# fnordware/j2k

Hardware: AMD Instinct MI355X
Metric: Mpixels/s encode, 8Kx8K 16-bit RGB, 5 DWT levels; DWT HBM GB/s vs roofline (higher is better)
Workload: dtype f32

## Files before the change

j2k_amd/csrc/encoder.cpp:

```cpp
#include <hip/hip_runtime.h>

#include <dlfcn.h>

#include <algorithm>
#include <atomic>
#include <chrono>
#include <condition_variable>
#include <functional>
#include <future>
#include <limits>
#include <cstdio>
#include <cstdlib>
#include <cstring>
#include <memory>
#include <mutex>
#include <thread>
#include <string>
#include <vector>

#include "common.h"
#include "geometry.h"
#include "kernels.h"
#include "tier2.h"
#include "jp2.h"
// ... 469 lines not shown
    std::unique_lock<std::mutex> dense(dev.dense);
    const unsigned dense_seq = ++dev.seq;
    unsigned *const dwt_word = dev.dwt_done_word;
    unsigned *const dwt_busy = (dwt_word && tn.mq_yield && tn.overlap && dev.inflight.load() > 1) ? dwt_word + 32 : nullptr;
    const size_t nb1 = g.cblks.size();
    const size_t nb = nb1 * F;
    const T1Tables tt(nb);
    e->sym.ensure(e->sym_bytes * F + 1024);
    e->out.ensure(e->out_bytes * F + 64);
    e->meta.ensure(tt.meta_bytes());
    e->passes.ensure(tt.passes_bytes());
    HIP_CHECK(hipMemsetAsync(tt.err(e->meta.as<uint32_t>()), 0, sizeof(uint32_t), s));

    const bool overlap_mq = tn.overlap != 0;
    if (overlap_mq && dev.last_dense_done && dev.last_dense_done != e->k1_done) HIP_CHECK(hipStreamWaitEvent(s, dev.last_dense_done, 0));
    HIP_CHECK(hipEventRecord(e->ev[EV_UPLOAD], s));

    const size_t plane_bytes = e->frame_elems * sizeof(int32_t);
    FrontendArgs fa0 = make_frontend_args(cod, dplanes, x0, y0, x1, y1);
    const bool fused = fuse_frontend(cod, fa0, tn);
    if (!fused || NL >= 3) e->P.ensure(plane_bytes * F);
    if (NL >= 1) e->Z.ensure(plane_bytes * F);
    if (NL >= 2) e->Q.ensure(plane_bytes * F);
    const bool level_events = tn.level_events != 0;
    double dwt_bytes = 0;
    struct BusyGuard {
        unsigned *word = nullptr; hipStream_t s;
        ~BusyGuard() { if (word) (void)hipMemsetAsync(word, 0, sizeof(unsigned), s); }
    } busy_guard;
    busy_guard.s = s;
    for (size_t f = 0; f < F; ++f) {
    if (f > 0) for (uint32_t c = 0; c < cod.ncomp; ++c) dplanes[c] = planes[f * cod.ncomp + c];
    FrontendArgs fa = f == 0 ? fa0 : make_frontend_args(cod, dplanes, x0, y0, x1, y1);
    if (!fused) {
        fa.dst_x0 = x0; fa.dst_y0 = y0;
        run_frontend(e, cod, fa, reinterpret_cast<int32_t *>(e->P.as<uint8_t>() + f * plane_bytes), e->comp_off, S, s);
    }
    if (f == 0) e->last_fa = fa;
    if (f == 0) HIP_CHECK(hipEventRecord(e->ev[EV_FRONT], s));

    if (f == 0 && dwt_busy && NL > 0) { launch_set_word(dwt_busy, 1u, s); busy_guard.word = dwt_busy; }
    const bool own_bracket = f == 0 && F == 1 && NL > 0 && tn.level1_dispatch_events;
    if (f == 0 && !own_bracket) HIP_CHECK(hipEventRecord(e->lev[0], s));
    for (int l = 0; l < NL; ++l) {
        const int l1 = l + 1;
        const bool last_own = own_bracket && !level_events && l > 0 && l == NL - 1;
        const bool bracketed = (l == 0 && own_bracket) || last_own;
        launch_dwt_levels(e, cod, fa, fused, f, l, l1, s, bracketed ? e->lev[l] : nullptr, bracketed ? e->lev[l1] : nullptr);
        HIP_CHECK(hipGetLastError());
        for (const DwtJob &j : e->h_jobs[(size_t)l]) dwt_bytes += 8.0 * j.rw * j.rh;
        if (!bracketed && ((F == 1 && level_events) || (l == 0 && F == 1) || (l1 == NL && f == F - 1))) HIP_CHECK(hipEventRecord(e->lev[l1], s));
        if (l == 0 && f == 0 && busy_guard.word && tn.mq_yield == 1 && NL > 1) { launch_set_word(dwt_busy, 0u, s); busy_guard.word = nullptr; }
    }
    }
    e->last_levels = NL;
    e->last_fused = fused;
    const bool word_by_modeller = dwt_word && !busy_guard.word;
    if (dwt_word && !word_by_modeller) launch_set_word(dwt_word, dense_seq, s, busy_guard.word, 0u);
    busy_guard.word = nullptr;
    HIP_CHECK(hipEventRecord(e->ev[EV_DWT], s));

    if (F > 1 && (e->seq_frames != F || !e->seq_valid)) {
        e->h_blks_seq.resize(nb);
        for (size_t f = 0; f < F; ++f)
            for (size_t i = 0; i < nb1; ++i) {
                CblkDev d = e->h_blks[i];
                d.coef_off += (unsigned long long)f * e->frame_elems;
                d.sym_off += (unsigned long long)f * e->sym_bytes;
                d.out_off += (unsigned long long)f * e->out_bytes;
                e->h_blks_seq[f * nb1 + i] = d;
            }
        e->blks_seq.ensure(nb * sizeof(CblkDev));
        HIP_CHECK(hipMemcpyAsync(e->blks_seq.p, e->h_blks_seq.data(), nb * sizeof(CblkDev), hipMemcpyHostToDevice, s));
        e->seq_frames = F; e->seq_valid = true;
    }
    const CblkDev *dblk = F > 1 ? e->blks_seq.as<CblkDev>() : e->blks.as<CblkDev>();
    uint32_t *meta = e->meta.as<uint32_t>();
    T1Args ta{};
    ta.coef = NL >= 1 ? e->Z.p : e->P.p; ta.stride = (long long)S;
    ta.blks = dblk; ta.nblks = (int)nb; ta.reversible = cod.reversible;
    t1_arena_args(e, tt, ta);
    ta.mq_prio = tn.mq_prio ? 3 : 0;
    ta.sparse = tn.t1_sparse;
    ta.style = cod.cblk_style;
#ifdef J2K_MQ_TIMES
    {
        static unsigned long long *dbg = nullptr;
        if (!dbg) { HIP_CHECK(hipMalloc(reinterpret_cast<void **>(&dbg), kT1Counters * 8)); }
        else {
            unsigned long long h[12];
            HIP_CHECK(hipMemcpy(h, dbg, sizeof(h), hipMemcpyDeviceToHost));
            const double ch = (double)std::max(1ull, h[4]), wv = (double)std::max(1ull, h[5]);
            std::fprintf(stderr, "coder waves (previous frame): %.0f workgroups, %.0f chunks each; per chunk of 16 decisions, counter ticks: producer work %.1f + barrier %.1f | "
                                 "consumer work %.1f + barrier %.1f\n", wv, ch / wv, h[0] / ch, h[1] / ch, h[2] / ch, h[3] / ch);
        }
        HIP_CHECK(hipMemset(dbg, 0, kT1Counters * 8));
        ta.dbg = dbg;
    }
#endif
#ifdef J2K_T1_COUNTERS
    t1_counters(ta);
#endif
    ta.yield_word = (dwt_word && tn.mq_yield && tn.overlap) ? dwt_word + 32 : nullptr;
    const bool rate_control = cod.rate_control();
    ta.want_dist = rate_control ? 1 : 0;
    ta.want_rates = rate_control ? 1 : 0;
    {
        const int big_groups = std::max(2, std::min(7, tn.groups));
        const int groups = nb >= 8192 ? big_groups : 1;
        int first = 0;
        for (int gi = 0; gi < groups; ++gi) {
            const size_t eighth = (nb / 8) / 64 * 64;
            int last = gi == groups - 1 ? (int)nb : (int)((eighth + (nb - eighth) * (size_t)gi / (size_t)(groups - 1)) / 64 * 64);
            T1Args tg = ta;
            tg.first = first; tg.nblks = last;
            if (gi == 0 && word_by_modeller) { tg.done_word = dwt_word; tg.done_value = dense_seq; }
            launch_t1_model(tg, s);
            {
                HIP_CHECK(hipEventRecord(e->gev[gi], s));
                HIP_CHECK(hipStreamWaitEvent(coder_stream(e, gi), e->gev[gi], 0));
                if (tn.mq_wait_us > 0 && dwt_word && overlap_mq && gi == groups - 1 && groups > 1 && dev.inflight.load() > 1)
                    launch_wait_word(dwt_word, dense_seq + 1, (unsigned)tn.mq_wait_us, e->mqs[gi]);
                launch_t1_mq(tg, e->mqs[gi]);
                HIP_CHECK(hipEventRecord(e->mq_done[gi], e->mqs[gi]));
            }
            first = last;
        }
        HIP_CHECK(hipEventRecord(e->k1_done, s));
        for (int gi = 0; gi < groups; ++gi) HIP_CHECK(hipStreamWaitEvent(s, e->mq_done[gi], 0));
    }
    HIP_CHECK(hipEventRecord(e->ev[EV_T1], s));

    e->h_meta.ensure(tt.meta_bytes());
    HIP_CHECK(hipMemcpyAsync(e->h_meta.p, meta, tt.meta_words() * sizeof(uint32_t), hipMemcpyDeviceToHost, s));
    if (rate_control && nb) {
        T1Args tf = ta;
        tf.first = 0; tf.nblks = (int)nb;
        launch_t1_rate_fixup(tf, s);
        e->h_passes.ensure(tt.h_passes_bytes());
        const int dev_min = tn.rate_dev == 0 ? 8192 : tn.rate_dev;
        pd.rc_device = dev_min > 0 && cod.psnr.empty() && F == 1 && nb >= (size_t)dev_min && (!cod.max_comp_size || dev.inflight.load() <= 1);
        pd.rc_tables_pending = false;
        if (!(pd.rc_device && tn.overlap))
            HIP_CHECK(hipMemcpyAsync(e->h_passes.p, ta.pass_nmsedec, tt.h_passes_bytes(), hipMemcpyDeviceToHost, s));
        if (pd.rc_device) {
            const RateArgs ra = rate_args(e, tt);
            if (!e->rc_weight_valid) {
                const std::vector<double> w = rate_block_weights(g);
                std::memcpy(e->h_rc_bounds.p, w.data(), nb * sizeof(double));
                unsigned char *hc = e->h_rc_bounds.as<unsigned char>() + nb * sizeof(double);
                for (size_t i = 0; i < nb; ++i) hc[i] = (unsigned char)std::min<uint32_t>(g.cblks[i].comp, 3u);
                HIP_CHECK(hipMemcpyAsync(e->rc_weight.p, e->h_rc_bounds.p, nb * sizeof(double) + nb, hipMemcpyHostToDevice, s));
                e->rc_weight_valid = true;
            }
            launch_rate_prepare(ra, s);
            if (tn.overlap) {
                hipStream_t side = coder_stream(e, 0);
                HIP_CHECK(hipEventRecord(e->rc_fixed, s));
                HIP_CHECK(hipStreamWaitEvent(side, e->rc_fixed, 0));
                HIP_CHECK(hipMemcpyAsync(e->h_passes.p, ta.pass_nmsedec, tt.h_passes_bytes(), hipMemcpyDeviceToHost, side));
                HIP_CHECK(hipEventRecord(e->rc_tables, side));
                pd.rc_tables_pending = true;
            }
            HIP_CHECK(hipMemcpyAsync(e->h_rc_bounds.p, ra.bounds, 3 * nb * sizeof(double), hipMemcpyDeviceToHost, s));
        }
    } else {
// ... 237 lines not shown
    for (int k = 0; k < j2k_hip_encoder::kMaxStages; ++k) {
        if (!e->stage_done[k]) HIP_CHECK(hipEventCreateWithFlags(&e->stage_done[k], hipEventDisableTiming));
        if (!e->stage_dl[k]) HIP_CHECK(hipEventCreateWithFlags(&e->stage_dl[k], hipEventDisableTiming));
    }
    if (!e->band_valid || e->band_row_end != rows) {
        e->band = build_band_schedule(g, rows, split_last);
        e->band_row_end = rows;
        e->h_blks_band.resize(nb);
        size_t sym_off = 0, out_off = 0;
        for (size_t n = 0; n < nb; ++n) {
            CblkDev d = e->h_blks[e->band.perm[n]];
            d.sym_off = sym_off; d.out_off = out_off;
            sym_off += d.sym_cap; out_off += d.out_cap;
            e->h_blks_band[n] = d;
        }
        e->blks_band.ensure(nb * sizeof(CblkDev));
        e->pack_dst.ensure(nb * sizeof(unsigned long long));
        HIP_CHECK(hipMemcpyAsync(e->blks_band.p, e->h_blks_band.data(), nb * sizeof(CblkDev), hipMemcpyHostToDevice, s));
        const BandSchedule &Sn = e->band;
        const int nst = (int)Sn.stages.size(), nbands = (int)rows.size();
        e->h_gate_groups.clear(); e->h_group_of.assign(nb, 0);
        e->stage_group_first.assign((size_t)nst, 0); e->stage_group_count.assign((size_t)nst, 0);
        for (int k = 0; k < nst; ++k) {
            const BandStage &st = Sn.stages[(size_t)k];
            e->stage_group_first[(size_t)k] = (uint32_t)e->h_gate_groups.size();
            const unsigned prio = (st.band == nbands - 1 && nbands > 1) ? 3u : (2 * st.band >= nbands - 1 ? 2u : 1u);
            for (uint32_t f = 0; f < st.blk_count; f += 64) {
                const uint32_t cnt = std::min<uint32_t>(64, st.blk_count - f);
                for (uint32_t i = 0; i < cnt; ++i) e->h_group_of[st.blk_first + f + i] = (uint32_t)e->h_gate_groups.size();
                e->h_gate_groups.push_back(T1Args::GateGroup{st.blk_first + f, cnt, (unsigned)k, prio});
            }
            e->stage_group_count[(size_t)k] = (uint32_t)e->h_gate_groups.size() - e->stage_group_first[(size_t)k];
        }
        e->gate_groups.ensure(std::max<size_t>(1, e->h_gate_groups.size()) * sizeof(T1Args::GateGroup));
        e->gate_group_of.ensure(nb * sizeof(uint32_t));
        if (!e->h_gate_groups.empty())
            HIP_CHECK(hipMemcpyAsync(e->gate_groups.p, e->h_gate_groups.data(), e->h_gate_groups.size() * sizeof(T1Args::GateGroup), hipMemcpyHostToDevice, s));
        HIP_CHECK(hipMemcpyAsync(e->gate_group_of.p, e->h_group_of.data(), nb * sizeof(uint32_t), hipMemcpyHostToDevice, s));
        HIP_CHECK(hipStreamSynchronize(s));
        e->band_valid = true;
    }
    const BandSchedule &S = e->band;
    const int NS = (int)S.stages.size();
    if (NS > j2k_hip_encoder::kMaxStages) throw Error(J2K_HIP_ERR_PARAM, "internal: more stages than events");
    const size_t NG = e->h_gate_groups.size();

    const size_t pad = reinterpret_cast<uintptr_t>(lo) & 15;
    e->in.ensure(span + pad + 16);
    uint8_t *const dbase = e->in.as<uint8_t>() + pad;
    const size_t plane_bytes = e->plane_elems * sizeof(int32_t) * cod.ncomp;
    if (NL >= 3) e->P.ensure(plane_bytes);
    e->Z.ensure(plane_bytes);
    if (NL >= 2) e->Q.ensure(plane_bytes);
    e->sym.ensure(e->sym_bytes + 1024);
    e->out.ensure(e->out_bytes + 64);
    e->cs.ensure(e->out_bytes + 64);
    const T1Tables tt(nb);
    e->meta.ensure(tt.meta_bytes());
    e->passes.ensure(tt.passes_bytes());
    e->h_meta.ensure(tt.meta_bytes());
    uint32_t *meta = e->meta.as<uint32_t>();
    e->gate_state.ensure((NG + (size_t)NS + 8) * sizeof(uint32_t));
    unsigned *const gate_ready = e->gate_state.as<unsigned>(), *const gate_done = gate_ready + NG, *const gate_abort = gate_done + NS;
    HIP_CHECK(hipEventRecord(e->ev[EV_START], s));
    HIP_CHECK(hipMemsetAsync(tt.err(meta), 0, sizeof(uint32_t), s));
    HIP_CHECK(hipMemsetAsync(gate_ready, 0, (NG + (size_t)NS + 8) * sizeof(uint32_t), s));
    HIP_CHECK(hipEventRecord(e->gates_zeroed, s));

    j2k_hip_plane dplanes[4];
    for (uint32_t c = 0; c < cod.ncomp; ++c) {
        dplanes[c] = planes[c];
        dplanes[c].base = dbase + (static_cast<const uint8_t *>(planes[c].base) - lo);
    }
    const FrontendArgs fa = make_frontend_args(cod, dplanes, 0, 0, (int)cod.width, (int)cod.height);
    e->last_fa = fa; e->last_fused = true; e->last_levels = NL;
    for (int l = 0; l < NL; ++l) e->level_ms[l] = 0;

    T1Args ta{};
    ta.coef = e->Z.p; ta.stride = (long long)e->stride;
    ta.blks = e->blks_band.as<CblkDev>(); ta.nblks = (int)nb; ta.reversible = cod.reversible;
    t1_arena_args(e, tt, ta);
    ta.mq_prio = tn.mq_prio ? 3 : 0;
    ta.sparse = tn.t1_sparse;
    ta.want_rates = 0;
    ta.gate_groups = e->gate_groups.as<T1Args::GateGroup>(); ta.gate_group_of = e->gate_group_of.as<unsigned>();
    ta.gate_ready = gate_ready; ta.gate_done = gate_done; ta.gate_abort = gate_abort;
    ta.gate_budget = 1u << 21;

    double dwt_bytes = 0;
    for (int l = 0; l < NL; ++l)
        for (const DwtJob &j : e->h_jobs[(size_t)l]) dwt_bytes += 8.0 * j.rw * j.rh;

    pd.banded = true;
    HIP_CHECK(hipStreamWaitEvent(s_coder, e->gates_zeroed, 0));
    for (size_t g0 = 0; g0 < NG; g0 += 1024) launch_t1_mq_gated(ta, (int)g0, (int)std::min<size_t>(1024, NG - g0), s_coder);
    double up_ms = 0;
    for (int k = 0; k < NS; ++k) {
        const BandStage &st = S.stages[(size_t)k];
        if (k < B) {
            Range r("j2k_hip upload band");
            const uint8_t *b0 = k ? lo + (size_t)rows[(size_t)k - 1] * (size_t)rowbytes : lo;
            const uint8_t *b1 = k == B - 1 ? hi : std::min(hi, lo + (size_t)rows[(size_t)k] * (size_t)rowbytes);
            const double t0 = now_ms();
            if (b1 > b0) HIP_CHECK(hipMemcpyAsync(dbase + (b0 - lo), b0, (size_t)(b1 - b0), hipMemcpyHostToDevice, e->up_stream));
            up_ms += now_ms() - t0;
            HIP_CHECK(hipEventRecord(e->band_up[k], e->up_stream));
        }
        Range r("j2k_hip band enqueue");
        if (k < B) HIP_CHECK(hipStreamWaitEvent(s, e->band_up[k], 0));
        for (const BandLaunch &bl : st.dwt) {
            DwtLevelArgs da = dwt_level_args(e, cod, fa, true, 0, (int)bl.level, (int)bl.tile_row);
            da.pair0 = bl.pair0; da.pair1 = bl.pair1;
            launch_dwt_level(da, s);
        }
        HIP_CHECK(hipGetLastError());
        if (k < B) {
            HIP_CHECK(hipEventRecord(e->gev[k], s));
            uint32_t first = st.blk_first, count = st.blk_count;
            if (k == B - 1) for (int q = B; q < NS; ++q) count += S.stages[(size_t)q].blk_count;
            if (count) {
                T1Args tg = ta;
                tg.first = (int)first; tg.nblks = (int)(first + count);
                tg.model_prio = (k == B - 1 && B > 1) ? 3 : 0;
                HIP_CHECK(hipStreamWaitEvent(s_model, e->gev[k], 0));
                launch_t1_model(tg, s_model);
            }
        }
    }
    HIP_CHECK(hipEventSynchronize(e->band_up[B - 1]));
    pd.t_uploaded = now_ms();
    for (int k = 0; k < NS; ++k) {
        const BandStage &st = S.stages[(size_t)k];
        if (st.blk_count) {
            launch_wait_count(gate_done + k, e->stage_group_count[(size_t)k], 10000000u, gate_abort, ta.err, e->dl_stream);
            unsigned long long *pd_dst = e->pack_dst.as<unsigned long long>() + st.blk_first;
            launch_pack_offsets(ta.len + st.blk_first, (int)st.blk_count, e->h_blks_band[st.blk_first].out_off, pd_dst, e->dl_stream);
            GatherArgs ga{};
            ga.dst = e->cs.as<uint8_t>(); ga.out = e->out.as<uint8_t>(); ga.blks = ta.blks + st.blk_first;
            ga.cblk_dst = pd_dst; ga.len = ta.len + st.blk_first; ga.nblks = (int)st.blk_count;
            launch_gather(ga, e->dl_stream);
            HIP_CHECK(hipMemcpy2DAsync(tt.numbps(e->h_meta.as<uint32_t>()) + st.blk_first, tt.column_bytes(), tt.numbps(meta) + st.blk_first, tt.column_bytes(),
                                       st.blk_count * sizeof(uint32_t), T1Tables::kColumns, hipMemcpyDeviceToHost, e->dl_stream));
        }
        HIP_CHECK(hipEventRecord(e->stage_done[k], e->dl_stream));
    }


    for (int k = 0; k < NS; ++k) HIP_CHECK(hipStreamWaitEvent(s, e->stage_done[k], 0));
    HIP_CHECK(hipMemcpyAsync(tt.err(e->h_meta.as<uint32_t>()), tt.err(meta), sizeof(uint32_t), hipMemcpyDeviceToHost, s));
    HIP_CHECK(hipEventRecord(e->ev[EV_T1], s));

    pd.active = true;
    pd.F = 1; pd.nb1 = nb; pd.framed = true; pd.rate_control = false; pd.dwt_bytes = dwt_bytes;
    pd.meta = meta; pd.dblk = ta.blks; pd.nl = NL;
    pd.banded = true; pd.stages = NS; pd.bands = B; pd.ms_upload_host = up_ms;
    return true;
}

struct PieceWriter {
    j2k_hip_write_fn write; void *user; std::vector<uint8_t> &bounce; size_t fill = 0;
    static constexpr size_t kSmall = 256u << 10, kBounce = 4u << 20;
    void out(const uint8_t *p, size_t n) { if (n && write(user, p, n) != n) throw Error(J2K_HIP_ERR_SINK, "Error writing file"); }
    void flush() { if (fill) { out(bounce.data(), fill); fill = 0; } }
    void put(const uint8_t *p, size_t n)
    {
        if (n >= kSmall) { flush(); out(p, n); return; }
// ... 673 lines not shown
```

j2k_amd/csrc/kernels.h:

```cpp
#pragma once

#include <hip/hip_runtime.h>

#include <cstdint>

#include "rgba_plan.h"

namespace j2k_hip {

struct Tuning {
    int overlap = 1;
    int no_fuse = 0;
    int level_events = 0;
    int level1_dispatch_events = 1;
    int mq_prio = 1;
    int mq_yield = 2;
    int groups = 2;
    int alloc_threads = 8;
    int rate_dev = 0;
    int rate_dev_scan = 0;
    int mq_wait_us = 1500;
    int dwt_pairs = 2;
    int dwt_ppc = 0;
    int dwt_min_waves = 2048;
    int fused_wpb = 0;
    int fused_ppc = 0;
    int fused_generic = 0;
    int dwt_xcd = 1;
    int t1dec_tail = 1;
    int t1dec_lanes = 1;
    int decseq_group = 0;
    int bands = 0;
    int t1_sparse = 0;
};
Tuning &tuning();
int tune(const char *key, int value);
int get_tune(const char *key, int *value);

struct FrontendArgs {
    const uint8_t *src[4];
    long long colbytes[4], rowbytes[4];
    int sample_bytes[4];
    int src_depth[4];
    int ncomp;
    int width;
    int x0;
    int y0, y1;
    int dst_x0, dst_y0;
    int prec;
    int reversible, mct, promote;
    int interleaved;
    const uint8_t *pixel_base;
    int pixel_bytes;
    int chan_off[4];
    void *dst[4];
    long long dst_stride;
    const float *xyz_lin[3];
    const float *xyz_thr;
    float xyz_m[9];
};
void launch_frontend(const FrontendArgs &a, hipStream_t s);
void launch_frontend_sycc(const FrontendArgs &a, int sub_x, int sub_y, hipStream_t s);
void launch_frontend_xyz(const FrontendArgs &a, hipStream_t s);

constexpr int kCompareWords = 8;
constexpr int kCompareSets = 16;
struct CompareArgs {
    FrontendArgs src;
    int wide;
    const int *planes[4]; long long plane_stride; int plane_dc;
    const uint16_t *dec[4]; long long dec_stride[4]; int dec_sx[4], dec_sy[4];
    int ncomp, width, height;
    int slot[4];
    unsigned long long *acc;
};
void launch_compare(const CompareArgs &a, hipStream_t s);

struct DwtJob {
    long long src_off;
    long long ll_off;
    long long z_off;
    int rw, rh;
    int casx, casy;
    int px0, py0;
};
struct DwtLevelArgs {
    const void *src; long long src_stride;
    void *ll; long long ll_stride;
    void *z; long long z_stride;
    const DwtJob *jobs; int njobs;
    int max_rw, max_rh;
    int reversible;
    int pair0, pair1;
    int shared_chip;
    int fused;
    long long comp_stride;
    struct Fused {
        const uint8_t *base;
        long long rowbytes;
        int pixb;
        int k0, k1, k2, k3;
        int rs;
        int dc;
        int mct;
        int ncomp;
        int promote;
        int src_depth, prec;
    } fe;
};
void launch_dwt_level(const DwtLevelArgs &a, hipStream_t s, hipEvent_t start = nullptr, hipEvent_t stop = nullptr);
int fused_occupancy(bool rev, int ncomp);
void launch_membw(const void *src, void *dst, int w, int h, int rows, int mode, hipStream_t s);

struct CblkDev {
    unsigned long long coef_off;
    unsigned long long sym_off;
    unsigned long long out_off;
    unsigned int sym_cap, out_cap;
    float stepsize;
    unsigned short w, h;
    unsigned char orient, Mb;
    unsigned char pad[2];
};
constexpr int kDevMaxPasses = 96;
constexpr int kT1Counters = 56;
struct T1Args {
    const void *coef; long long stride;
    const CblkDev *blks; int nblks;
    int first;
    int reversible;
    int want_dist;
    int want_rates;
    int mq_prio;
    int model_prio;
    int sparse;
#if defined(J2K_T1_COUNTERS) || defined(J2K_MQ_TIMES)
    unsigned long long *dbg;
#endif
    unsigned *done_word; unsigned done_value;
    struct GateGroup { unsigned first, count, stage, prio; };
    const GateGroup *gate_groups;
    const unsigned *gate_group_of;
    unsigned *gate_ready, *gate_done;
    const unsigned *gate_abort;
    unsigned gate_budget;
    const unsigned *yield_word;
    uint8_t *sym;
    uint8_t *out;
    unsigned int *numbps, *npasses, *nsym, *len, *err;
    unsigned int *pass_nsym;
    int *pass_nmsedec;
    unsigned int *pass_rate;
    unsigned style;
};
void launch_t1_model(const T1Args &a, hipStream_t s);
void launch_t1_mq(const T1Args &a, hipStream_t s);
void launch_t1_mq_styled(const T1Args &a, hipStream_t s);
void launch_t1_mq_gated(const T1Args &a, int group_first, int group_count, hipStream_t s);
void launch_wait_count(const unsigned *word, unsigned target, unsigned timeout_us, const unsigned *abort, unsigned *err, hipStream_t s);
void launch_wait_word(const unsigned *word, unsigned target, unsigned timeout_us, hipStream_t s);
void launch_set_word(unsigned *word, unsigned value, hipStream_t s, unsigned *word2 = nullptr, unsigned value2 = 0);
void launch_t1_rate_fixup(const T1Args &a, hipStream_t s);

struct Taken;
struct RateArgs {
    unsigned nblks;
    const double *weight;
    const unsigned char *comp_of;
    const unsigned *numbps, *npasses;
    const int *pass_nmsedec;
    const unsigned *pass_rate;
    double *disto;
    float *reach;
    double *bounds;
    const unsigned char *done;
    const double *ahead;
    long long *delta;
    unsigned *scan_bytes;
    Taken *scan_taken;
    unsigned long long *scan_sums;
};
void launch_rate_prepare(const RateArgs &a, hipStream_t s);
void launch_rate_ahead(const RateArgs &a, unsigned first, unsigned count, unsigned K, hipStream_t s);
void launch_rate_scan(const RateArgs &a, unsigned first, unsigned count, double thresh, hipStream_t s);

struct DecBlkDev {
    unsigned long long cw_off;
    unsigned long long mask_off;
    unsigned long long coef_off;
    unsigned int cw_len;
    float stepsize;
    unsigned short w, h, npasses;
    unsigned char orient, numbps;
    unsigned int seg_off;
    unsigned short nsegs;
    unsigned char roishift;
};
struct DecGroupDev {
    unsigned long long plane_off;
    unsigned maxpasses, maxstripes;
};
struct T1DecArgs {
    const uint8_t *cw;
    unsigned long long *masks;
    void *coef; long long stride;
    const DecBlkDev *blks; int nblks;
    int reversible;
    const DecGroupDev *groups;
    unsigned *state, *planes;
    const unsigned *cwsegs;
    unsigned style;
#ifdef T1L_STATS
    unsigned long long *stats;
#endif
};
void launch_t1_decode(const T1DecArgs &a, hipStream_t s);
void launch_t1_decode_lanes(const T1DecArgs &a, hipStream_t s);
int t1_decode_lanes_resident_waves();

struct IdwtJob {
    long long off;
    int rw, rh;
    int casx, casy;
};
struct IdwtArgs {
    void *a, *tmp; long long stride;
    const IdwtJob *jobs; int njobs;
    int max_rw, max_rh;
    int reversible;
};
void launch_idwt_level(const IdwtArgs &a, hipStream_t s);

struct IdwtWinJob {
    long long off;
    int rw, rh, casx, casy;
    int wx0, wx1, wy0, wy1;
// ... 52 lines not shown
```

j2k_amd/csrc/stage_hooks.cpp:

```cpp
#include <algorithm>
#include <cstring>
#include <memory>
#include <string>
#include <utility>
#include <vector>

#include "cblk_style.h"
#include "handle.h"
#include "rate_device.h"
#include "tier2.h"

using namespace j2k_hip;

static int stage_t1_blocks(j2k_hip_encoder *e, int reversible, void *d_coef, uint32_t stride, uint32_t nblocks,
                           const uint32_t *bx, const uint32_t *by, const uint32_t *bw, const uint32_t *bh, const uint32_t *orient,
                           const float *stepsize, uint32_t *numbps, uint32_t *npasses, uint32_t *length, uint64_t *offsets,
                           void *data, size_t data_cap, uint32_t *pass_rate, int32_t *pass_dist, uint32_t cblk_style)
{
    if (!e) return J2K_HIP_ERR_PARAM;
    return guarded(e, [&] {
        if (e->pend.active) throw Error(J2K_HIP_ERR_PARAM, "the previous j2k_hip_encode_begin on this handle has not been finished");
        if (cblk_style & kStyleVcausal) throw Error(J2K_HIP_ERR_PARAM, "cblk_style: vertically causal contexts (bit 8) are not written");
        if (cblk_style & ~(uint32_t)(kStylesEncoded | kStyleVcausal)) throw Error(J2K_HIP_ERR_PARAM, "cblk_style: unknown code-block style bits");
        HIP_CHECK(hipSetDevice(e->device));
        hipStream_t s = e->stream;
        const size_t nb = nblocks;
        std::vector<CblkDev> blks(nb);
        size_t sym_off = 0, out_off = 0;
        for (size_t i = 0; i < nb; ++i) {
            if (bw[i] == 0 || bh[i] == 0 || bw[i] > 64 || bh[i] > 64 || orient[i] > 3) throw Error(J2K_HIP_ERR_PARAM, "bad code-block rectangle");
            CblkDev d{};
            d.coef_off = (unsigned long long)by[i] * stride + bx[i];
            const size_t area = (size_t)bw[i] * bh[i];
            const CblkCaps caps = cblk_capacities(area, 30, cblk_style);
            const size_t symcap = caps.sym, outcap = caps.out;
            d.sym_off = sym_off; d.sym_cap = (unsigned)symcap; d.out_off = out_off; d.out_cap = (unsigned)outcap;
            d.stepsize = stepsize ? stepsize[i] : 1.0f;
            d.w = (unsigned short)bw[i]; d.h = (unsigned short)bh[i]; d.orient = (unsigned char)orient[i]; d.Mb = 30;
            sym_off += symcap; out_off += outcap;
            blks[i] = d;
        }
        {
            std::vector<uint32_t> order(nb);
            for (uint32_t i = 0; i < nb; ++i) order[i] = i;
            std::sort(order.begin(), order.end(), [&](uint32_t a, uint32_t b) { return by[a] < by[b]; });
            for (size_t i = 0; i < nb; ++i)
                for (size_t j = i + 1; j < nb && by[order[j]] < by[order[i]] + bh[order[i]]; ++j) {
                    const uint32_t a = order[i], b = order[j];
                    if (bx[a] < bx[b] + bw[b] && bx[b] < bx[a] + bw[a]) throw Error(J2K_HIP_ERR_PARAM, "code-block rectangles overlap");
                }
            for (size_t i = 0; i < nb; ++i)
                if ((uint64_t)bx[i] + bw[i] > stride) throw Error(J2K_HIP_ERR_PARAM, "code-block rectangle wider than the plane's stride");
        }
        invalidate_cached_tables(e);
        const T1Tables tt(nb);
        e->blks.ensure(std::max<size_t>(1, nb) * sizeof(CblkDev));
        if (nb) HIP_CHECK(hipMemcpyAsync(e->blks.p, blks.data(), nb * sizeof(CblkDev), hipMemcpyHostToDevice, s));
        e->sym.ensure(sym_off + 1024); e->out.ensure(out_off + 64);
        e->meta.ensure(tt.meta_bytes());
        e->passes.ensure(tt.passes_bytes());
        T1Args ta{};
        ta.coef = d_coef; ta.stride = stride; ta.blks = e->blks.as<CblkDev>(); ta.nblks = (int)nb; ta.reversible = reversible;
        t1_arena_args(e, tt, ta);
        ta.want_dist = pass_dist != nullptr;
        ta.want_rates = pass_rate || pass_dist;
        ta.sparse = tuning().t1_sparse;
        ta.style = cblk_style;
#ifdef J2K_T1_COUNTERS
        t1_counters(ta);
#endif
        HIP_CHECK(hipMemsetAsync(ta.err, 0, sizeof(uint32_t), s));
        launch_t1_model(ta, s);
        launch_t1_mq(ta, s);
        if (cblk_style) launch_t1_rate_fixup(ta, s);
        std::vector<uint32_t> hm(tt.meta_words());
        HIP_CHECK(hipMemcpyAsync(hm.data(), e->meta.p, hm.size() * sizeof(uint32_t), hipMemcpyDeviceToHost, s));
        HIP_CHECK(hipStreamSynchronize(s));
        if (*tt.err(hm.data())) throw Error(J2K_HIP_ERR_OVERFLOW, "Tier-1 kernel reported error " + std::to_string(*tt.err(hm.data())));
        size_t pos = 0;
        for (size_t i = 0; i < nb; ++i) {
            numbps[i] = tt.numbps(hm.data())[i]; npasses[i] = tt.npasses(hm.data())[i]; length[i] = tt.len(hm.data())[i];
            offsets[i] = pos;
            if (pos + length[i] > data_cap) throw Error(J2K_HIP_ERR_OVERFLOW, "data buffer too small");
            if (length[i]) HIP_CHECK(hipMemcpy(static_cast<uint8_t *>(data) + pos, e->out.as<uint8_t>() + blks[i].out_off, length[i], hipMemcpyDeviceToHost));
            pos += length[i];
        }
        if (pass_rate || pass_dist) {
            std::vector<uint32_t> hp(tt.passes_words());
            HIP_CHECK(hipMemcpy(hp.data(), e->passes.p, hp.size() * sizeof(uint32_t), hipMemcpyDeviceToHost));
            for (size_t i = 0; i < nb; ++i) {
                const uint32_t np = npasses[i];
                uint32_t *rate = tt.pass_rate(hp.data()) + tt.row(i);
                const uint32_t *nmsedec = tt.pass_nmsedec(hp.data()) + tt.row(i);
                if (!cblk_style) {
                    uint32_t last = length[i];
                    for (uint32_t p = np; p > 0;) { --p; if (rate[p] > last) rate[p] = last; else last = rate[p]; }
                    const uint8_t *bytes = static_cast<const uint8_t *>(data) + offsets[i];
                    for (uint32_t p = 0; p < np; ++p)
                        if (rate[p] > 0 && bytes[rate[p] - 1] == 0xff) --rate[p];
                }
                for (uint32_t p = 0; p < (uint32_t)kDevMaxPasses; ++p) {
                    if (pass_rate) pass_rate[tt.row(i) + p] = p < np ? rate[p] : 0;
                    if (pass_dist) pass_dist[tt.row(i) + p] = p < np ? (int32_t)nmsedec[p] : 0;
                }
            }
        }
    });
}

extern "C" {

int j2k_hip_stage_frontend(j2k_hip_encoder *e, const j2k_hip_params *params, const j2k_hip_plane *planes_device, void *d_out)
{
    if (!e) return J2K_HIP_ERR_PARAM;
    return guarded(e, [&] {
        if (e->pend.active) throw Error(J2K_HIP_ERR_PARAM, "the previous j2k_hip_encode_begin on this handle has not been finished");
        HIP_CHECK(hipSetDevice(e->device));
        const Coding cod = normalise(params);
        FrontendArgs fa = make_frontend_args(cod, planes_device, 0, 0, (int)cod.width, (int)cod.height);
        if (cod.subsampled() || cod.rgb_to_sycc || cod.rgb_to_xyz) {
            const PlaneLayout lay = plane_layout(cod, 0, 0, (int)cod.width, (int)cod.height);
            e->P.ensure(lay.frame_elems * sizeof(int32_t));
            run_frontend(e, cod, fa, e->P.as<int32_t>(), lay.comp_off, lay.stride, e->stream);
            HIP_CHECK(hipGetLastError());
            uint8_t *out = static_cast<uint8_t *>(d_out);
            for (uint32_t c = 0; c < cod.ncomp; ++c) {
                const size_t cw = (size_t)lay.cw[c], chh = (size_t)lay.ch[c];
                HIP_CHECK(hipMemcpy2DAsync(out, cw * 4, e->P.as<int32_t>() + lay.comp_off[c], lay.stride * 4, cw * 4, chh, hipMemcpyDeviceToDevice, e->stream));
                out += cw * chh * 4;
            }
            HIP_CHECK(hipStreamSynchronize(e->stream));
            return;
        }
        for (uint32_t c = 0; c < cod.ncomp; ++c) fa.dst[c] = static_cast<int32_t *>(d_out) + (size_t)c * cod.width * cod.height;
        fa.dst_stride = cod.width;
        launch_frontend(fa, e->stream);
        HIP_CHECK(hipStreamSynchronize(e->stream));
    });
}

int j2k_hip_stage_dwt(j2k_hip_encoder *e, int reversible, uint32_t width, uint32_t height, uint32_t nplanes, uint32_t levels,
                      uint32_t x0, uint32_t y0, const void *d_in, void *d_out, uint32_t repeat, double *ms_out)
{
    if (!e) return J2K_HIP_ERR_PARAM;
    return guarded(e, [&] {
        if (e->pend.active) throw Error(J2K_HIP_ERR_PARAM, "the previous j2k_hip_encode_begin on this handle has not been finished");
        HIP_CHECK(hipSetDevice(e->device));
        if (!width || !height || !nplanes || levels > 32) throw Error(J2K_HIP_ERR_PARAM, "bad DWT stage arguments");
        const size_t plane = (size_t)width * height;
// ... 575 lines not shown
```

j2k_amd/csrc/t1.hip:

```cpp
#include "kernels.h"
#include "t1_common.h"
#include "cblk_style.h"

#include <algorithm>
#include <cstdlib>
#include <type_traits>

namespace j2k_hip {
namespace {


constexpr int kFrac = 6;
constexpr int kFlush = 1024;
constexpr int kStageBytes = kFlush + 64 * 10;


__device__ __forceinline__ void set_priority(int p)
{
    if (p >= 3) __builtin_amdgcn_s_setprio(3);
    else if (p == 2) __builtin_amdgcn_s_setprio(2);
    else if (p == 1) __builtin_amdgcn_s_setprio(1);
}

__device__ __forceinline__ unsigned from_left(unsigned v) { return (unsigned)__builtin_amdgcn_update_dpp(0, (int)v, 0x138 , 0xf, 0xf, false); }
__device__ __forceinline__ unsigned from_right(unsigned v) { return (unsigned)__builtin_amdgcn_update_dpp(0, (int)v, 0x130 , 0xf, 0xf, false); }

__device__ __forceinline__ u64 from_left64(u64 v) { return (u64)from_left((unsigned)v) | ((u64)from_left((unsigned)(v >> 32)) << 32); }
__device__ __forceinline__ u64 from_right64(u64 v) { return (u64)from_right((unsigned)v) | ((u64)from_right((unsigned)(v >> 32)) << 32); }

__device__ __forceinline__ unsigned prefix_count_dpp(unsigned cnt, unsigned &total)
{
    int t = (int)cnt;
    t += __builtin_amdgcn_update_dpp(0, t, 0x111, 0xf, 0xf, false);
    t += __builtin_amdgcn_update_dpp(0, t, 0x112, 0xf, 0xf, false);
    t += __builtin_amdgcn_update_dpp(0, t, 0x114, 0xf, 0xf, false);
    t += __builtin_amdgcn_update_dpp(0, t, 0x118, 0xf, 0xf, false);
    t += __builtin_amdgcn_update_dpp(0, t, 0x142, 0xa, 0xf, false);
    t += __builtin_amdgcn_update_dpp(0, t, 0x143, 0xc, 0xf, false);
    total = (unsigned)__builtin_amdgcn_readlane(t, 63);
    return (unsigned)t - cnt;
}

__device__ __forceinline__ unsigned nibble_counts(unsigned v)
{
    const unsigned x = v - ((v >> 1) & 0x55555555u);
    return (x & 0x33333333u) + ((x >> 2) & 0x33333333u);
}

constexpr unsigned kDenseStripe = 103, kSparseHead = 64, kSparseRound = 44;
constexpr unsigned kBurst = 64 * 10;

__device__ __forceinline__ int nmsedec_sig(unsigned m, int bp)
{
    const int i = (int)((m >> bp) & 127u);
    return bp > 0 ? max(0, (3 * i - 144) * 128) : ((i * i + 32) >> 6) * 128;
}
__device__ __forceinline__ int nmsedec_ref(unsigned m, int bp)
{
    const int i = (int)((m >> bp) & 127u);
    if (bp > 0) return i >= 64 ? max(0, (i - 80) * 128) : max(0, (48 - i) * 128);
    return (((i - 64) * (i - 64) + 32) >> 6) * 128;
}

struct PackSel {
    u64 v[256];
    constexpr PackSel() : v()
    {
        for (int e = 0; e < 256; ++e) {
            u64 sel = 0x0c0c0c0c0c0c0c0cull;
            int k = 0;
            for (int r = 0; r < 4; ++r) {
                if ((e >> r) & 1) { sel = (sel & ~(0xffull << (8 * k))) | ((u64)r << (8 * k)); ++k; }
                if ((e >> (4 + r)) & 1) { sel = (sel & ~(0xffull << (8 * k))) | ((u64)(4 + r) << (8 * k)); ++k; }
            }
            v[e] = sel;
        }
    }
};
__constant__ PackSel kPackSel = PackSel();

struct PairTab {
    unsigned v[256];
    constexpr PairTab() : v()
    {
        for (unsigned e = 0; e < 256; ++e) {
// ... 693 lines not shown
#ifdef J2K_MQ_TIMES
        long long tw_ = 0, tb_ = 0;
#endif
        for (unsigned c = 0; c <= nchunks; ++c) {
#ifdef J2K_MQ_TIMES
            const long long t0_ = __builtin_readcyclecounter();
#endif
            if (a.yield_word && (c & 3u) == 0) {
                while (yield_budget && __builtin_amdgcn_readfirstlane((int)__hip_atomic_load(a.yield_word, __ATOMIC_RELAXED, __HIP_MEMORY_SCOPE_AGENT))) {
                    __builtin_amdgcn_s_sleep(64);
                    --yield_budget;
                }
            }
            if (c < nchunks) {
                const unsigned base = c * 16;
                const uint4 chunk = next;
                if (base + 16 < nsym) next = *reinterpret_cast<const uint4 *>(sym + base + 16);
                const unsigned words[4] = {chunk.x, chunk.y, chunk.z, chunk.w};
                const int rem = (int)min(nsym - min(base, nsym), 16u);
                unsigned char *const ctx_b = reinterpret_cast<unsigned char *>(ctxs);
                const unsigned char *const trans_b = reinterpret_cast<const unsigned char *>(trans);
                const unsigned lane4 = (unsigned)lane * 4u;
                auto decide = [&](unsigned c4, unsigned b4, auto jj_) -> unsigned {
                    constexpr unsigned jj = decltype(jj_)::value;
                    unsigned *const cp = reinterpret_cast<unsigned *>(ctx_b + __builtin_amdgcn_perm(c4, lane4, 0x0c0c0400u + (jj << 8)));
                    const unsigned st = *cp;
                    const unsigned ta = (st ^ __builtin_amdgcn_perm(b4, 0u, 0x0c0c040cu + (jj << 8))) & 0x3fcu;
                    const unsigned tr = *reinterpret_cast<const unsigned *>(trans_b + ta);
                    const bool mps = ta < (1u << kMq2LpsBit);
                    const unsigned qe = st & 0xffff0000u;
                    const unsigned A1 = A - qe;
                    const bool use_a1 = (A1 >= qe) == mps;
                    A = use_a1 ? A1 : qe;
                    const bool renorm = (int)A >= 0;
                    *cp = renorm ? tr : st;
                    const unsigned n = (unsigned)__builtin_clz(A);
                    A <<= n;
                    return __builtin_amdgcn_alignbit(n, use_a1 ? qe : 0u, 16);
                };
                if (__all(rem == 16)) {
#pragma unroll
                    for (int g = 0; g < 4; ++g) {
                        const unsigned c4 = (words[g] >> 1) & 0x1f1f1f1fu, b4 = words[g] << 1;
                        unsigned e[4];
                        e[0] = decide(c4, b4, std::integral_constant<unsigned, 0>());
                        e[1] = decide(c4, b4, std::integral_constant<unsigned, 1>());
                        e[2] = decide(c4, b4, std::integral_constant<unsigned, 2>());
                        e[3] = decide(c4, b4, std::integral_constant<unsigned, 3>());
                        queue[c & 1][g][lane] = make_uint4(e[0], e[1], e[2], e[3]);
                    }
                } else
#pragma unroll
                for (int g = 0; g < 4; ++g) {
                    const unsigned c4 = (words[g] >> 1) & 0x1f1f1f1fu, b4 = words[g] << 1;
                    unsigned e[4] = {0, 0, 0, 0};
                    if (4 * g + 0 < rem) e[0] = decide(c4, b4, std::integral_constant<unsigned, 0>());
                    if (4 * g + 1 < rem) e[1] = decide(c4, b4, std::integral_constant<unsigned, 1>());
                    if (4 * g + 2 < rem) e[2] = decide(c4, b4, std::integral_constant<unsigned, 2>());
                    if (4 * g + 3 < rem) e[3] = decide(c4, b4, std::integral_constant<unsigned, 3>());
                    queue[c & 1][g][lane] = make_uint4(e[0], e[1], e[2], e[3]);
                }
            } else {
                finalA[lane] = A >> 16;
            }
#ifdef J2K_MQ_TIMES
            const long long t1_ = __builtin_readcyclecounter();
            __syncthreads();
            tw_ += t1_ - t0_; tb_ += __builtin_readcyclecounter() - t1_;
#else
            __syncthreads();
#endif
        }
#ifdef J2K_MQ_TIMES
        if (lane == 0 && a.dbg) { atomicAdd(a.dbg + 0, (unsigned long long)tw_); atomicAdd(a.dbg + 1, (unsigned long long)tb_); atomicAdd(a.dbg + 4, (unsigned long long)nchunks); atomicAdd(a.dbg + 5, 1ull); }
#endif
        return;
    }

    unsigned char *out = a.out + cb.out_off;
    const unsigned *pass_nsym = a.pass_nsym + (size_t)(live ? b : 0) * kDevMaxPasses;
    unsigned *pass_rate = a.pass_rate + (size_t)(live ? b : 0) * kDevMaxPasses;
    unsigned char *ostage_b = reinterpret_cast<unsigned char *>(ostage);
    unsigned C = 0, CT = 12, B = 0;
    int flushed = 0;
    bool overflow = false;
    const unsigned dbase = (unsigned)lane * (kRing + 4u) + 4u;
    unsigned pos = dbase - 1u;
    auto nbytes = [&]() -> int { return (int)(pos - dbase) + flushed; };
    auto byteout = [&](bool p) {
        const bool was_ff = B == 0xffu;
        const unsigned Bc = B + ((C > 0x7ffffffu && !was_ff) ? 1u : 0u);
        const bool stuff = Bc == 0xffu;
        const unsigned sh = stuff ? 20u : 19u, ct = 27u - sh;
        const unsigned bw = was_ff ? 8u : ct;
        ostage_b[pos] = (unsigned char)Bc;
        B = p ? __builtin_amdgcn_ubfe(C, sh, bw) : B; C = p ? __builtin_amdgcn_ubfe(C, 0u, sh) : C; CT = p ? ct : CT; pos += p ? 1u : 0u;
        asm("" : "+v"(pos));
    };
    unsigned cur_pass = 0;
    unsigned next_end = 0xffffffffu;
    if constexpr (RATES) next_end = npasses ? pass_nsym[0] : 0xffffffffu;
    auto close_passes = [&](unsigned i) {
        while (cur_pass < npasses && i == next_end) {
            pass_rate[cur_pass] = (unsigned)(nbytes() + 3);
            ++cur_pass;
            next_end = cur_pass < npasses ? pass_nsym[cur_pass] : 0xffffffffu;
        }
    };
#ifdef J2K_MQ_TIMES
    long long tw_ = 0, tb_ = 0;
#endif
    for (unsigned c = 0; c <= nchunks; ++c) {
#ifdef J2K_MQ_TIMES
        const long long t0_ = __builtin_readcyclecounter();
#endif
        if (c >= 1) {
            const unsigned base = (c - 1) * 16;
            int rel = 64;
            if constexpr (RATES) rel = (int)min(next_end - base, 64u);
            auto four = [&](auto check, const unsigned (&e)[4], const int g) {
                constexpr bool ENDS = decltype(check)::value;
                {
#pragma unroll
                    for (int jj = 0; jj < 4; ++jj) {
                        const int j = 4 * g + jj;
                        C += e[jj] & 0xffffu;
                        unsigned n = e[jj] >> 16;
                        {
                            const bool p = n >= CT;
                            const unsigned k = p ? CT : 0u;
                            C <<= k; n -= k;
                            byteout(p);
                        }
                        if (__any(n >= CT)) {
                            const bool p2 = n >= CT;
                            const unsigned k2 = p2 ? CT : 0u;
                            C <<= k2; n -= k2;
                            byteout(p2);
                            if (__any(n >= CT)) {
                                const bool p3 = n >= CT;
                                const unsigned k3 = p3 ? CT : 0u;
                                C <<= k3; n -= k3;
                                byteout(p3);
                            }
                        }
                        C <<= n; CT -= n;
                        if constexpr (ENDS) {
                            if (rel == j + 1) { close_passes(base + j + 1); rel = (int)min(next_end - base, 64u); }
                        }
                    }
                }
            };
            bool ends_here = false;
            if constexpr (RATES) ends_here = __any(rel <= 16);
#pragma unroll
            for (int g = 0; g < 4; ++g) {
                const uint4 q = queue[(c - 1) & 1][g][lane];
                const unsigned e[4] = {q.x, q.y, q.z, q.w};
                if constexpr (RATES) {
                    if (ends_here && __any(rel > 4 * g && rel <= 4 * g + 4)) four(std::true_type(), e, g);
                    else four(std::false_type(), e, g);
                } else four(std::false_type(), e, g);
            }
            const int waiting = (int)(pos - dbase);
            if (__any(waiting >= 64)) {
                const int units = waiting >> 4;
                for (int u = 0; u < 7; ++u) {
                    if (!__any(u < units)) break;
                    if (u < units) {
                        if ((unsigned)(flushed + 16) <= cb.out_cap) {
                            const unsigned *sp = reinterpret_cast<const unsigned *>(ostage_b + dbase + 16 * u);
                            *reinterpret_cast<uint4 *>(out + flushed) = make_uint4(sp[0], sp[1], sp[2], sp[3]);
                        } else overflow = true;
                        flushed += 16;
                    }
                }
                if (units > 0) {
                    const unsigned *sp = reinterpret_cast<const unsigned *>(ostage_b + dbase + 16 * units);
                    unsigned *dp = reinterpret_cast<unsigned *>(ostage_b + dbase);
                    const unsigned r0 = sp[0], r1 = sp[1], r2 = sp[2], r3 = sp[3];
                    dp[0] = r0; dp[1] = r1; dp[2] = r2; dp[3] = r3;
                    pos -= 16u * (unsigned)units;
                }
            }
        }
#ifdef J2K_MQ_TIMES
        const long long t1_ = __builtin_readcyclecounter();
        __syncthreads();
        tw_ += t1_ - t0_; tb_ += __builtin_readcyclecounter() - t1_;
#else
        __syncthreads();
#endif
    }
#ifdef J2K_MQ_TIMES
    if (lane == 0 && a.dbg) { atomicAdd(a.dbg + 2, (unsigned long long)tw_); atomicAdd(a.dbg + 3, (unsigned long long)tb_); }
#endif
    const bool fin = live && npasses;
    const unsigned A = finalA[lane];
    if (fin) {
        if constexpr (RATES) close_passes(nsym);
        const unsigned tempc = C + A;
        C |= 0xffffu;
        if (C >= tempc) C -= 0x8000u;
    }
    C <<= CT; byteout(fin);
    C <<= CT; byteout(fin);
    if (fin && B != 0xffu) {
        ostage_b[pos] = (unsigned char)B;
        ++pos;
    }
    const int nb = nbytes();
    if (fin) {
        for (int o = flushed; o < nb; o += 4) {
            if ((unsigned)(o + 4) <= cb.out_cap) *reinterpret_cast<unsigned *>(out + o) = *reinterpret_cast<const unsigned *>(ostage_b + dbase + (o - flushed));
            else overflow = true;
        }
        if constexpr (RATES) pass_rate[npasses - 1] = (unsigned)nb;
        a.len[b] = (unsigned)nb;
        if (overflow) a.err[0] = 3u;
    } else if (live) {
        a.len[b] = 0;
    } else if (a.gate_groups && lane < (int)gg.count) {
        a.len[b] = 0;
    }
    if (a.gate_groups) {
        __builtin_amdgcn_fence(__ATOMIC_RELEASE, "agent");
        if (lane == 0) __hip_atomic_fetch_add(a.gate_done + gg.stage, 1u, __ATOMIC_RELEASE, __HIP_MEMORY_SCOPE_AGENT);
    }
}

__global__ void t1_rate_fixup_kernel(T1Args a)
{
    const int b = a.first + (int)(blockIdx.x * blockDim.x + threadIdx.x);
    if (b >= a.nblks) return;
    const unsigned np = a.npasses[b];
    unsigned *rate = a.pass_rate + (size_t)b * kDevMaxPasses;
    const unsigned char *bytes = a.out + a.blks[b].out_off;
    unsigned last = a.len[b];
    for (unsigned p = np; p > 0;) { --p; if (rate[p] > last) rate[p] = last; else last = rate[p]; }
    for (unsigned p = 0; p < np; ++p)
        if (rate[p] > 0 && bytes[rate[p] - 1] == 0xffu) --rate[p];
}

__global__ void wait_word_kernel(const unsigned *word, unsigned target, unsigned timeout_us)
{
    for (unsigned i = 0; i < timeout_us; ++i) {
        if ((int)(__hip_atomic_load(word, __ATOMIC_RELAXED, __HIP_MEMORY_SCOPE_AGENT) - target) >= 0) return;
        __builtin_amdgcn_s_sleep(32);
    }
}

__global__ void wait_count_kernel(const unsigned *word, unsigned target, unsigned timeout_us, const unsigned *abort, unsigned *err)
{
    for (unsigned i = 0; i < timeout_us; i += 2) {
        if (__hip_atomic_load(word, __ATOMIC_ACQUIRE, __HIP_MEMORY_SCOPE_AGENT) >= target) return;
        if (abort && __hip_atomic_load(abort, __ATOMIC_RELAXED, __HIP_MEMORY_SCOPE_AGENT)) break;
        __builtin_amdgcn_s_sleep(64);
    }
    if (threadIdx.x == 0) *err = 5u;
}

__global__ void set_word_kernel(unsigned *word, unsigned value, unsigned *word2, unsigned value2)
{
    if (threadIdx.x == 0) {
        if (word2) __hip_atomic_store(word2, value2, __ATOMIC_RELAXED, __HIP_MEMORY_SCOPE_AGENT);
        __hip_atomic_store(word, value, __ATOMIC_RELAXED, __HIP_MEMORY_SCOPE_AGENT);
    }
}

}

void launch_wait_word(const unsigned *word, unsigned target, unsigned timeout_us, hipStream_t s)
{
    hipLaunchKernelGGL(wait_word_kernel, dim3(1), dim3(64), 0, s, word, target, timeout_us);
}

void launch_wait_count(const unsigned *word, unsigned target, unsigned timeout_us, const unsigned *abort, unsigned *err, hipStream_t s)
{
    hipLaunchKernelGGL(wait_count_kernel, dim3(1), dim3(64), 0, s, word, target, timeout_us, abort, err);
// ... 50 lines not shown
```

j2k_amd/csrc/tuning.cpp:

```cpp
#include <cstdlib>
#include <cstring>
#include <mutex>

#include "kernels.h"

namespace j2k_hip {
namespace {

struct Knob { const char *key; const char *env; int Tuning::*field; };
const Knob kKnobs[] = {
    {"overlap", nullptr, &Tuning::overlap},
    {"no_fuse", "J2K_NO_FUSE", &Tuning::no_fuse},
    {"level_events", "J2K_DWT_LEVEL_EVENTS", &Tuning::level_events},
    {"mq_prio", "J2K_MQ_PRIO", &Tuning::mq_prio},
    {"level1_dispatch_events", "J2K_LEVEL1_DISPATCH_EVENTS", &Tuning::level1_dispatch_events},
    {"groups", "J2K_GROUPS", &Tuning::groups},
    {"mq_wait_us", "J2K_MQ_WAIT_US", &Tuning::mq_wait_us},
    {"dwt_pairs", "J2K_DWT_PAIRS", &Tuning::dwt_pairs},
    {"mq_yield", "J2K_MQ_YIELD", &Tuning::mq_yield},
    {"alloc_threads", "J2K_ALLOC_THREADS", &Tuning::alloc_threads},
    {"rate_dev", "J2K_RATE_DEV", &Tuning::rate_dev},
    {"rate_dev_scan", "J2K_RATE_DEV_SCAN", &Tuning::rate_dev_scan},
    {"dwt_ppc", "J2K_DWT_PPC", &Tuning::dwt_ppc},
    {"dwt_min_waves", "J2K_DWT_MIN_WAVES", &Tuning::dwt_min_waves},
    {"fused_wpb", "J2K_DWT_FUSED_WPB", &Tuning::fused_wpb},
    {"fused_ppc", "J2K_DWT_FUSED_PPC", &Tuning::fused_ppc},
    {"fused_generic", "J2K_DWT_FUSED_GENERIC", &Tuning::fused_generic},
    {"dwt_xcd", "J2K_DWT_XCD", &Tuning::dwt_xcd},
    {"t1dec_lanes", "J2K_T1DEC_LANES", &Tuning::t1dec_lanes},
    {"t1dec_tail", "J2K_T1DEC_TAIL", &Tuning::t1dec_tail},
    {"decseq_group", "J2K_DECSEQ_GROUP", &Tuning::decseq_group},
    {"bands", "J2K_BANDS", &Tuning::bands},
    {"t1_sparse", "J2K_T1_SPARSE", &Tuning::t1_sparse},
};

Tuning g_tuning;
std::once_flag g_once;

void from_env()
{
    for (const Knob &k : kKnobs) {
        if (!k.env) continue;
        const char *v = std::getenv(k.env);
        if (v && *v) g_tuning.*(k.field) = std::atoi(v);
        else if (v && (k.field == &Tuning::no_fuse || k.field == &Tuning::level_events))
            g_tuning.*(k.field) = 1;
    }
    if (std::getenv("J2K_NO_OVERLAP")) g_tuning.overlap = 0;
}

}

Tuning &tuning()
{
    std::call_once(g_once, from_env);
    return g_tuning;
}

int tune(const char *key, int value)
{
    if (!key) return 1;
    Tuning &t = tuning();
    for (const Knob &k : kKnobs)
        if (std::strcmp(k.key, key) == 0) { t.*(k.field) = value; return 0; }
    return 1;
}

int get_tune(const char *key, int *value)
{
    if (!key || !value) return 1;
    Tuning &t = tuning();
    for (const Knob &k : kKnobs)
        if (std::strcmp(k.key, key) == 0) { *value = t.*(k.field); return 0; }
    return 1;
}

}
```

Baseline: 10740.

## Add wide-register windowed MQ byte-out path with fallback to exact coder

```diff
diff --git a/j2k_amd/csrc/encoder.cpp b/j2k_amd/csrc/encoder.cpp
--- a/j2k_amd/csrc/encoder.cpp
+++ b/j2k_amd/csrc/encoder.cpp
@@ -575,6 +575,7 @@
     t1_arena_args(e, tt, ta);
     ta.mq_prio = tn.mq_prio ? 3 : 0;
     ta.sparse = tn.t1_sparse;
+    ta.mq_window = tn.mq_window;
     ta.style = cod.cblk_style;
 #ifdef J2K_MQ_TIMES
     {
@@ -978,6 +979,7 @@
     t1_arena_args(e, tt, ta);
     ta.mq_prio = tn.mq_prio ? 3 : 0;
     ta.sparse = tn.t1_sparse;
+    ta.mq_window = tn.mq_window;
     ta.want_rates = 0;
     ta.gate_groups = e->gate_groups.as<T1Args::GateGroup>(); ta.gate_group_of = e->gate_group_of.as<unsigned>();
     ta.gate_ready = gate_ready; ta.gate_done = gate_done; ta.gate_abort = gate_abort;
diff --git a/j2k_amd/csrc/kernels.h b/j2k_amd/csrc/kernels.h
--- a/j2k_amd/csrc/kernels.h
+++ b/j2k_amd/csrc/kernels.h
@@ -32,6 +32,7 @@
     int decseq_group = 0;
     int bands = 0;
     int t1_sparse = 0;
+    int mq_window = 0;
 };
 Tuning &tuning();
 int tune(const char *key, int value);
@@ -152,6 +153,7 @@
     int *pass_nmsedec;
     unsigned int *pass_rate;
     unsigned style;
+    int mq_window;
 };
 void launch_t1_model(const T1Args &a, hipStream_t s);
 void launch_t1_mq(const T1Args &a, hipStream_t s);
diff --git a/j2k_amd/csrc/stage_hooks.cpp b/j2k_amd/csrc/stage_hooks.cpp
--- a/j2k_amd/csrc/stage_hooks.cpp
+++ b/j2k_amd/csrc/stage_hooks.cpp
@@ -65,6 +65,7 @@
         ta.want_dist = pass_dist != nullptr;
         ta.want_rates = pass_rate || pass_dist;
         ta.sparse = tuning().t1_sparse;
+        ta.mq_window = tuning().mq_window;
         ta.style = cblk_style;
 #ifdef J2K_T1_COUNTERS
         t1_counters(ta);
diff --git a/j2k_amd/csrc/t1.hip b/j2k_amd/csrc/t1.hip
--- a/j2k_amd/csrc/t1.hip
+++ b/j2k_amd/csrc/t1.hip
@@ -1,6 +1,7 @@
 #include "kernels.h"
 #include "t1_common.h"
 #include "cblk_style.h"
+#include "t1_mq_window.h"
 
 #include <algorithm>
 #include <cstdlib>
@@ -860,6 +861,9 @@
     unsigned *pass_rate = a.pass_rate + (size_t)(live ? b : 0) * kDevMaxPasses;
     unsigned char *ostage_b = reinterpret_cast<unsigned char *>(ostage);
     unsigned C = 0, CT = 12, B = 0;
+    bool window = false, window_again = false;
+    if constexpr (!RATES) { window = a.mq_window >= 0; window_again = a.mq_window == 2; }
+    MqWide wide = mq_wide_from(C, CT, B);
     int flushed = 0;
     bool overflow = false;
     const unsigned dbase = (unsigned)lane * (kRing + 4u) + 4u;
@@ -938,6 +942,26 @@
                 if constexpr (RATES) {
                     if (ends_here && __any(rel > 4 * g && rel <= 4 * g + 4)) four(std::true_type(), e, g);
                     else four(std::false_type(), e, g);
+                } else if (window) {
+                    const MqWide wide0 = wide;
+                    const unsigned pos0 = pos;
+#pragma unroll
+                    for (int jj = 0; jj < 4; ++jj) mq_wide_add(wide, e[jj]);
+                    bool again = window_again || mq_wide_is_wide(wide) || mq_wide_has_carry(wide);
+                    if (!__any(again)) {
+                        while (__any(mq_wide_due(wide))) {
+                            const bool due = mq_wide_due(wide);
+                            const unsigned byte = mq_wide_peel(wide, due, again);
+                            ostage_b[pos] = (unsigned char)byte;
+                            pos += due ? 1u : 0u;
+                        }
+                    }
+                    if (__any(again)) {
+                        pos = pos0;
+                        mq_wide_to(wide0, C, CT, B);
+                        four(std::false_type(), e, g);
+                        wide = mq_wide_from(C, CT, B);
+                    }
                 } else four(std::false_type(), e, g);
             }
             const int waiting = (int)(pos - dbase);
@@ -973,6 +997,9 @@
 #ifdef J2K_MQ_TIMES
     if (lane == 0 && a.dbg) { atomicAdd(a.dbg + 2, (unsigned long long)tw_); atomicAdd(a.dbg + 3, (unsigned long long)tb_); }
 #endif
+    if constexpr (!RATES) {
+        if (window) mq_wide_to(wide, C, CT, B);
+    }
     const bool fin = live && npasses;
     const unsigned A = finalA[lane];
     if (fin) {
diff --git a/j2k_amd/csrc/t1_mq_window.h b/j2k_amd/csrc/t1_mq_window.h
--- /dev/null
+++ b/j2k_amd/csrc/t1_mq_window.h
@@ -0,0 +1,59 @@
+#pragma once
+
+#if defined(__HIPCC__)
+#define J2K_WIN_HD __host__ __device__ __forceinline__
+#else
+#define J2K_WIN_HD inline
+#endif
+
+namespace j2k_hip {
+
+struct MqWide {
+    unsigned long long V;
+    unsigned w;
+};
+
+constexpr unsigned kMqWideDue = 8u + 27u;
+constexpr unsigned kMqWideMax = 63u;
+
+J2K_WIN_HD MqWide mq_wide_from(unsigned C, unsigned CT, unsigned B)
+{
+    MqWide s;
+    s.V = ((unsigned long long)B << (27u - CT)) + C;
+    s.w = kMqWideDue - CT;
+    return s;
+}
+J2K_WIN_HD void mq_wide_to(const MqWide &s, unsigned &C, unsigned &CT, unsigned &B)
+{
+    const unsigned k = s.w - 8u;
+    const unsigned top = (unsigned)(s.V >> k), over = top >> 8;
+    CT = kMqWideDue - s.w;
+    B = top - over;
+    C = ((unsigned)s.V & ((1u << k) - 1u)) | (over << k);
+}
+
+J2K_WIN_HD void mq_wide_add(MqWide &s, unsigned e)
+{
+    const unsigned n = e >> 16;
+    s.V = (s.V + (e & 0xffffu)) << n;
+    s.w += n;
+}
+
+J2K_WIN_HD bool mq_wide_is_wide(const MqWide &s) { return s.w > kMqWideMax; }
+J2K_WIN_HD bool mq_wide_has_carry(const MqWide &s) { return (s.V >> (s.w & 63u)) != 0; }
+
+J2K_WIN_HD bool mq_wide_due(const MqWide &s) { return s.w >= kMqWideDue; }
+J2K_WIN_HD unsigned mq_wide_peel(MqWide &s, bool p, bool &rolled)
+{
+    const unsigned k = s.w - 8u;
+    const unsigned byte = (unsigned)(s.V >> k);
+    const unsigned long long rest = s.V - ((unsigned long long)byte << k);
+    const unsigned w1 = s.w - (byte == 0xffu ? 7u : 8u);
+    const bool zero = (rest >> (w1 - 8u)) == 0;
+    s.V = p ? rest : s.V;
+    s.w = p ? w1 : s.w;
+    rolled = rolled || (p && zero);
+    return byte;
+}
+
+}
diff --git a/j2k_amd/csrc/tuning.cpp b/j2k_amd/csrc/tuning.cpp
--- a/j2k_amd/csrc/tuning.cpp
+++ b/j2k_amd/csrc/tuning.cpp
@@ -32,6 +32,7 @@
     {"decseq_group", "J2K_DECSEQ_GROUP", &Tuning::decseq_group},
     {"bands", "J2K_BANDS", &Tuning::bands},
     {"t1_sparse", "J2K_T1_SPARSE", &Tuning::t1_sparse},
+    {"mq_window", "J2K_MQ_WINDOW", &Tuning::mq_window},
 };
 
 Tuning g_tuning;
```

After: 11460 (median of 6 runs). +6.8%, better.
